# sebastianffx/stainlib

Hardware: AMD Instinct MI355X
Metric: 1024x1024 H&E tiles/sec normalized (Macenko) (higher is better)
Workload: dtype f32; 1 GPU; configs[1]: batch of 512 tiles 1024x1024x3 uint8 per GPU, Macenko transform (fit once outside the timed region), tiles resident in HBM; tiles_per_gpu=512, failed_tiles=0

## Files before the change

stainlib_amd/csrc/stats_finish.hpp:

```cpp
#pragma once
#include "stats_selection.hpp"
#include "stats_sweeps.hpp"

namespace sl {

struct SampleAngleKey {
    const uint32_t* sample; TabView tab; float V[6]; int cps_log2; int P; float ylimf;
    __device__ __forceinline__ float operator()(int b) const {
        if (sample_absent(b, cps_log2, P)) return nan_f();
        return of_word(sample[b]);
    }
    __device__ __forceinline__ float of_word(uint32_t s) const {
        const uint32_t r = s & 255u, g = (s >> 8) & 255u, bl = (s >> 16) & 255u;
        const bool tissue = is_tissue_f(tab.gam(r), tab.gam(g), tab.gam(bl), ylimf);
        const float k = angle_key(V, tab.odf(r), tab.odf(g), tab.odf(bl));
        return tissue ? k : nan_f();
    }
    __device__ __forceinline__ bool present(int b, int n_sample) const { return b < n_sample && !sample_absent(b, cps_log2, P); }
};
struct SampleConcKey {
    const uint32_t* sample; TabView tab; LassoK L; int cps_log2; int P; int col;
    __device__ __forceinline__ void both(int b, float& c1, float& c2) const {
        if (sample_absent(b, cps_log2, P)) { c1 = c2 = nan_f(); return; }
        of_word(sample[b], c1, c2);
// ... 173 lines not shown
        uint32_t best = 0xffffffffu;
        float kn[U];
#pragma unroll
        for (int u = 0; u < U; ++u) { const int i = tid + u * bd; kn[u] = as_global(cand)[i < n ? i : 0]; }
        for (int i0 = tid; i0 < n; i0 += U * bd) {
            float k[U];
#pragma unroll
            for (int u = 0; u < U; ++u) {
                k[u] = kn[u];
                const int i = i0 + (U + u) * bd;
                kn[u] = as_global(cand)[i < n ? i : 0];
            }
#pragma unroll
            for (int u = 0; u < U; ++u) {
                if (i0 + u * bd >= n) continue;
                const int kb = pick_bin(k[u], ps.lo[b], ps.sc[b]);
                if (kb == (int)bin[b]) { const uint32_t pos = atomicAdd(&S.misc[24 + b], 1u); if (pos < 512u) list[512 * b + pos] = k[u]; }
                else if (kb > (int)bin[b]) best = min(best, f2ord(k[u]));
            }
        }
        for (int o = 32; o > 0; o >>= 1) best = min(best, (uint32_t)__shfl_xor((int)best, o, 64));
        if (lane == 0 && best != 0xffffffffu) atomicMin(&S.misc[26 + b], best);
    }
    __syncthreads();
    if (tid < 4) S.misc[28 + tid] = 0;
    __syncthreads();
#pragma unroll
    for (int b = 0; b < 2; ++b) {
        if (!done[b]) continue;
        const uint32_t m = cnt[b], ra = krel[b] - below[b];
        if ((uint32_t)tid < m) {
            const float me = list[512 * b + tid];
            uint32_t r = 0;
            for (uint32_t j = 0; j < m; ++j) {
                const float o = list[512 * b + j];
                r += (o < me || (o == me && j < (uint32_t)tid)) ? 1u : 0u;
            }
            if (r == ra) S.misc[28 + 2 * b] = __float_as_uint(me);
            if (r == ra + 1) S.misc[29 + 2 * b] = __float_as_uint(me);
        }
    }
    __syncthreads();
#pragma unroll
    for (int b = 0; b < 2; ++b) {
        if (!done[b]) continue;
        xa[b] = __uint_as_float(S.misc[28 + 2 * b]);
        const bool same_bin = krel[b] - below[b] + 1 < cnt[b];
        const uint32_t nx = S.misc[26 + b];
        xb[b] = same_bin ? __uint_as_float(S.misc[29 + 2 * b]) : (nx != 0xffffffffu ? ord2f(nx) : xa[b]);
    }
    __syncthreads();
}

template <bool TWO_COLS, class TileKeyAt>
__device__ __forceinline__ void stage_pick2(const float* cand0, const float* cand1, const uint32_t* n_in, uint32_t cap_list, bool complete,
                                            const float* lo, const float* hi, const long long* lt, int P, TileKeyAt tile_key_at, uint32_t n,
                                            const long long* k, const PickScale& ps, float* res , int& fallbacks, SelScratch& S) {
    bool fast[2], has2[2];
    uint32_t krel[2];
#pragma unroll
    for (int b = 0; b < 2; ++b) {
        const long long k2 = (k[b] + 1 < (long long)n) ? k[b] + 1 : k[b];
        has2[b] = k2 != k[b];
        const bool covered = complete && k[b] >= lt[b] && k2 < lt[b] + (long long)n_in[b];
        fast[b] = covered && lo[b] < hi[b] && n_in[b] <= cap_list;
        krel[b] = fast[b] ? (uint32_t)(k[b] - lt[b]) : 0u;
    }
    float xa[2] = {0, 0}, xb[2] = {0, 0};
    bool done[2] = {false, false};
    if (fast[0] | fast[1]) wg_pick2(cand0, cand1, n_in, fast, krel, ps, xa, xb, done, S);
#pragma unroll
    for (int b = 0; b < 2; ++b) {
        if (done[b]) {
            if (!has2[b]) xb[b] = xa[b];
        } else {
            if constexpr (TWO_COLS) tile_key_at.col = b;
            stage_order_stats(b ? cand1 : cand0, n_in[b], cap_list, complete, lo[b], hi[b], lt[b], P, tile_key_at, n, k[b], xa[b], xb[b], fallbacks, S);
        }
        res[2 * b] = xa[b]; res[2 * b + 1] = xb[b];
    }
}

__device__ __noinline__ void raw_flush(uint32_t buf_lds, uint32_t n, uint32_t* dst, unsigned int* head, uint32_t cap) {
#if defined(__HIP_DEVICE_COMPILE__)
    SL_LDS const uint32_t* buf = (SL_LDS const uint32_t*)buf_lds;
#else
    const uint32_t* buf = nullptr;
#endif
    const int lane = threadIdx.x & 63;
    uint32_t base = 0;
    if (lane == 0) base = atomicAdd(head, n);
    base = __builtin_amdgcn_readfirstlane(base);
    for (uint32_t i = lane; i < n; i += 64)
        if (base + i < cap) as_global(dst)[base + i] = buf[i];
}

struct RawSink {
    uint32_t buf;
    uint32_t n;
    uint32_t* dst;
    unsigned int* head;
    unsigned int* overflow;
    uint32_t cap;
    uint32_t stage_cap;
    __device__ __forceinline__ void flush(int) {
        if (n != 0) raw_flush(buf, n, dst, head, cap);
        n = 0;
    }
    __device__ __forceinline__ void put(unsigned long long m, const Chunk& ch, int px, int lane) {
        put_value(m, chunk_pixel(ch, px) & 0xffffffu, lane);
    }
    __device__ __forceinline__ void put_value(unsigned long long m, uint32_t value, int lane) {
        const uint32_t cnt = (uint32_t)__popcll(m);
        if (__builtin_expect(n + cnt > stage_cap, 0)) flush(lane);
        const uint32_t rank = __builtin_amdgcn_mbcnt_hi((uint32_t)(m >> 32), __builtin_amdgcn_mbcnt_lo((uint32_t)m, 0u));
#if defined(__HIP_DEVICE_COMPILE__)
        uint32_t sbase;
        asm("s_lshl2_add_u32 %0, %1, %2" : "=s"(sbase) : "s"(n), "s"(buf) : "scc");
        const uint32_t addr = sbase + 4u * rank;
        unsigned long long saved;
        asm volatile("s_mov_b64 %0, exec\n\ts_mov_b64 exec, %1\n\tds_write_b32 %2, %3\n\ts_mov_b64 exec, %0"
                     : "=&s"(saved) : "s"(m), "v"(addr), "v"(value) : "memory");
#else
        (void)rank; (void)value;
#endif
        n += cnt;
    }
};


// ... 211 lines not shown
```

stainlib_amd/csrc/stats_fused.hpp:

```cpp
#pragma once
#include "stats_phase_kernels.hpp"
#include "stats_cube.hpp"
#include "stats_twosweep.hpp"

namespace sl {

struct FusedArgs {
    const uint8_t* rgb;
    uint8_t* out;
    int n_tiles;
    int P;
    int stride_log2;
    int n_sample;
    float ylimf;
    double lam;
    double pct;
    const double* M_tgt;
    const double* maxC_tgt;
    int cap_raw, cap_list;
    uint32_t* raw;
    int cap_ang;
    uint32_t* raw_ang;
    float* cand;
    uint32_t* sample;
// ... 12 lines not shown
    int32_t* sweeps_out;
    int use_cube;
    int32_t* cube_out;
    int two_sweep;
    int sample_cap;
    int cl_lines;
    int cl_scale_log2;
    int32_t* ts_out;
    unsigned long long* next_tile;
};

template <int NT>
struct FusedShared {
    RowTab tab;
    uint32_t stage[NT / 64][kStageWave];
    SelScratch S;
    alignas(8) unsigned int n_raw;
    unsigned int n_ang;
    unsigned int overflow;
    double red[NT / 64][32];
    double sum[32];
    DictIter it;
    double Vd[6];
    double M[6];
    double maxC[2];
    float Vf[6];
    float lo[2], hi[2];
    float box[4];
    float res[4];
    LassoK L;
    int status;
    int conc_done;
    float xmin;
    int why;
    int use_cube;
    MergedConc mk;
    TwoSweep ts;
    int next_tile;
};

template <int NT>
struct FusedLds {
    static constexpr uint32_t tab = 0u;
    static constexpr uint32_t stage = (uint32_t)sizeof(RowTab);
    static constexpr uint32_t stage_wave = 4u * (uint32_t)kStageWave;
    static constexpr uint32_t hist = (uint32_t)(sizeof(RowTab) + sizeof(uint32_t) * (NT / 64) * kStageWave);
};
template <int NT>
__device__ __forceinline__ void fused_lds_origin(const FusedShared<NT>& sh) {
    static_assert(offsetof(FusedShared<NT>, tab) == FusedLds<NT>::tab && offsetof(FusedShared<NT>, stage) == FusedLds<NT>::stage &&
                  offsetof(FusedShared<NT>, S) == FusedLds<NT>::hist && offsetof(SelScratch, hist) == 0, "");
    if (lds_address(&sh) != 0u) __builtin_trap();
}

#define SL_FINISH_ATTR __noinline__
#ifdef SL_DEBUG_SUBCLK
#define SL_SUB_AT(clk, j) { __syncthreads(); if ((clk) && tid == 0) (clk)[(j)] = wall_clock64(); }
#else
#define SL_SUB_AT(clk, j)
#endif
#define SL_SUB(j) SL_SUB_AT(subclk, j)
template <class T>
__device__ __forceinline__ T* uni_ptr(T* p) {
    const unsigned long long v = (unsigned long long)(uintptr_t)p;
    const uint32_t lo = (uint32_t)__builtin_amdgcn_readfirstlane((int)(uint32_t)v), hi = (uint32_t)__builtin_amdgcn_readfirstlane((int)(uint32_t)(v >> 32));
    return (T*)(uintptr_t)(((unsigned long long)hi << 32) | lo);
}
__device__ __forceinline__ double uni_d(double x) {
    const unsigned long long v = (unsigned long long)__double_as_longlong(x);
    const uint32_t lo = (uint32_t)__builtin_amdgcn_readfirstlane((int)(uint32_t)v), hi = (uint32_t)__builtin_amdgcn_readfirstlane((int)(uint32_t)(v >> 32));
    return __longlong_as_double((long long)(((unsigned long long)hi << 32) | lo));
}

template <int NT>
__device__ SL_FINISH_ATTR void fused_cube_build(FusedShared<NT>* shp, uint32_t* samp_, int n_sample_, int cps_log2_, int P_, float ylimf_, int want_cube_) {
    FusedShared<NT>& sh = *shp;
    uint32_t* samp = uni_ptr(samp_);
    const int n_sample = __builtin_amdgcn_readfirstlane(n_sample_), cps_log2 = __builtin_amdgcn_readfirstlane(cps_log2_), P = __builtin_amdgcn_readfirstlane(P_);
    const int want_cube = __builtin_amdgcn_readfirstlane(want_cube_);
    const float ylimf = uni(ylimf_);
    const int tid = threadIdx.x;
    float* ctab = reinterpret_cast<float*>(&sh.stage[0][0]);
    static_assert(sizeof(sh.stage) >= sizeof(float) * kCubeTabFloats && sizeof(sh.S.hist) >= 4 * kCubeWords, "");
    const CubeConsts cc = cube_tables(view_of_b(sh.tab), sh.Vf, sh.hi[0], sh.lo[1], sh.mk, ctab, tid);
    __syncthreads();
    int share_pct;
    const bool pays = cube_worthwhile<NT>(samp, n_sample, cps_log2, P, ctab, cc, ylimf, &sh.S.misc[33], tid, share_pct);
    const bool go = pays || want_cube == 2;
    if (tid == 0) sh.use_cube = (go ? 1 : 0) | (share_pct << 8);
    if (go) cube_mask<NT>(ctab, cc, ylimf, sh.S.hist, tid);
    __syncthreads();
}

template <int NT>
__device__ SL_FINISH_ATTR void fused_finish1(FusedShared<NT>* shp, uint32_t* samp_, int n_sample_, int stride_log2_, int P_, float ylimf_, double pct_, double lam_,
                                           long long* subclk_, int want_cube_) {
    FusedShared<NT>& sh = *shp;
    uint32_t* samp = uni_ptr(samp_);
    const int n_sample = __builtin_amdgcn_readfirstlane(n_sample_), P = __builtin_amdgcn_readfirstlane(P_);
    const int sl2 = __builtin_amdgcn_readfirstlane(stride_log2_);
    const bool dense = sl2 < 0;
    const int stride_log2 = dense ? -sl2 : sl2;
    const int cps_log2 = dense ? kDenseCps : stride_log2 - 2;
    const float zs = dense ? (float)sqrt(kClusterDeff) : 1.0f;
    const int want_cube = __builtin_amdgcn_readfirstlane(want_cube_);
    const float ylimf = uni(ylimf_);
// ... 175 lines not shown
                                               float ylimf_, int stream_) {
    FusedShared<NT>& sh = *shp;
    const uint8_t* src = uni_ptr(src_);
    uint32_t* rawl = uni_ptr(rawl_);
    uint32_t* rawa = uni_ptr(rawa_);
    const int P = __builtin_amdgcn_readfirstlane(P_), cap_raw = __builtin_amdgcn_readfirstlane(cap_raw_), stream = __builtin_amdgcn_readfirstlane(stream_);
    const int cap_ang = __builtin_amdgcn_readfirstlane(cap_ang_);
    const float ylimf = uni(ylimf_);
    const int tid = threadIdx.x, wave = tid >> 6;
    const TabReaderB TB = TabReaderB::make_at(FusedLds<NT>::tab);
    const int nch = (P + 3) >> 2;
    SelConsts K;
    for (int i = 0; i < 6; ++i) K.V[i] = in_vgpr(sh.Vf[i]);
    K.L.g12 = 0.0f;
    K.xmin = -INFINITY;
#pragma unroll
    for (int i = 0; i < 2; ++i) {
        K.u[i][0] = in_vgpr(sh.mk.u[i][0]); K.u[i][1] = in_vgpr(sh.mk.u[i][1]); K.kt[i] = in_vgpr(sh.mk.kt[i]);
        K.eps[i] = in_vgpr(sh.mk.eps[i]); K.thr[i] = in_vgpr(sh.mk.thr[i]);
    }
    K.lo0 = uni(sh.lo[0]); K.hi0 = uni(sh.hi[0]); K.lo1 = uni(sh.lo[1]); K.hi1 = uni(sh.hi[1]);
    static_assert(offsetof(FusedShared<NT>, n_ang) == offsetof(FusedShared<NT>, n_raw) + 4 && offsetof(FusedShared<NT>, n_raw) % 8 == 0, "");
    const RawDirect direct{rawl, rawa, reinterpret_cast<unsigned long long*>(&sh.n_raw), (uint32_t)cap_raw, (uint32_t)cap_ang};
    static_assert(offsetof(FusedShared<NT>, S) % 4096 == 0 && offsetof(SelScratch, hist) == 0, "the cube mask must be 4 KB aligned");
    const uint32_t bits_lds = FusedLds<NT>::hist;
    const uint32_t ring_lds = (uint32_t)__builtin_amdgcn_readfirstlane((int)(FusedLds<NT>::stage + (uint32_t)wave * FusedLds<NT>::stage_wave));
    int t, c0, c1;
    fused_geometry<NT>(nch, tid, t, c0, c1);
    if (c0 >= c1) return;
    if (stream) select_sweep_cube<ALIGNED, kFusedTrip, true>(src, P, c0, c1, t, kFusedThreads, TB, ylimf, K, bits_lds, ring_lds, direct);
    else select_sweep_cube<ALIGNED, kFusedTrip, false>(src, P, c0, c1, t, kFusedThreads, TB, ylimf, K, bits_lds, ring_lds, direct);
}

template <int NT>
__device__ SL_FINISH_ATTR int fused_finish2(FusedShared<NT>* shp, const uint8_t* src_, uint32_t* rawl_, uint32_t* rawa_, float* cand0_, float* cand1_, int P_,
                                          int cap_raw_, int cap_ang_, int cap_list_, float ylimf_, double pct_, double lam_, long long* subclk_, int ts_ = 0) {
    FusedShared<NT>& sh = *shp;
    const uint8_t* src = uni_ptr(src_);
    uint32_t* rawl = uni_ptr(rawl_);
    uint32_t* rawa = uni_ptr(rawa_);
    const int cap_ang = __builtin_amdgcn_readfirstlane(cap_ang_);
    float* cand0 = uni_ptr(cand0_);
    float* cand1 = uni_ptr(cand1_);
    const int P = __builtin_amdgcn_readfirstlane(P_), cap_raw = __builtin_amdgcn_readfirstlane(cap_raw_), cap_list = __builtin_amdgcn_readfirstlane(cap_list_);
    const float ylimf = uni(ylimf_);
    const double pct = uni_d(pct_), lam = uni_d(lam_);
    long long* subclk = uni_ptr(subclk_);
    const int ts = __builtin_amdgcn_readfirstlane(ts_);
    const int tid = threadIdx.x, wave = tid >> 6;
    int fallbacks = 0;
    (void)subclk;
    const uint32_t T = (uint32_t)sh.sum[0];
    long long k[2];
    double gfrac[2];
    percentile_pos((double)T, 100.0 - pct, k[0], gfrac[0]);
    percentile_pos((double)T, pct, k[1], gfrac[1]);
    fin_tab_build(sh.tab);
    const FinTab FT{FusedLds<NT>::tab};
    const uint32_t stage_lds = FusedLds<NT>::tab + kFinTabBytes + (uint32_t)wave * fin_stage_bytes(NT);
    const uint32_t stage_entries = fin_stage_bytes(NT) / 8u;
    AngleTileKey tkey;
    tkey.src = src; tkey.tab = FT.view(); tkey.ylimf = ylimf;
    WordAngleKey rkey;
    rkey.T = FT; rkey.ylimf = ylimf;
    for (int i = 0; i < 6; ++i) { tkey.V[i] = sh.Vf[i]; rkey.V[i] = sh.Vf[i]; }
    const bool complete = sh.n_raw <= (uint32_t)cap_raw && sh.overflow == 0;
    const uint32_t n_raw = sh.n_raw < (uint32_t)cap_raw ? sh.n_raw : (uint32_t)cap_raw;
    const bool split = rawa != nullptr;
    const bool complete_a = split ? sh.n_ang <= (uint32_t)cap_ang : complete;
    const uint32_t n_a = split ? (sh.n_ang < (uint32_t)cap_ang ? sh.n_ang : (uint32_t)cap_ang) : n_raw;
    const uint32_t* lista = split ? rawa : rawl;
    const float los[2] = {sh.lo[0], sh.lo[1]}, his[2] = {sh.hi[0], sh.hi[1]};
    SL_SUB(2);
    const RefineOut ra = wg_refine_s(lista, (int)n_a, rkey, los[0], his[0], los[1], his[1], cand0, cand1, (uint32_t)cap_list, stage_lds,
                                     stage_entries, sh.S);
    SL_SUB(3);
    {
        const long long lt[2] = {(long long)ra.n_lt[0], (long long)T - (long long)ra.n_valid + (long long)ra.n_lt[1]};
        if (ts) {
            bool covered = complete_a;
#pragma unroll
            for (int b = 0; b < 2; ++b) {
                const long long k2 = (k[b] + 1 < (long long)T) ? k[b] + 1 : k[b];
                covered = covered & (k[b] >= lt[b]) & (k2 < lt[b] + (long long)ra.n_in[b]) & (ra.n_in[b] <= (uint32_t)cap_list);
            }
            if (!covered) {
                fin_tab_expand<NT>(sh.tab);
                return -1;
            }
        }
        float res[4];
        stage_pick2<false>(cand0, cand1, ra.n_in, (uint32_t)cap_list, complete_a, los, his, lt, P, tkey, T, k, ra.ps, res, fallbacks, sh.S);
        if (tid == 0) { sh.res[0] = res[0]; sh.res[1] = res[1]; sh.res[2] = res[2]; sh.res[3] = res[3]; }
        __syncthreads();
    }
    SL_SUB(5);
    if (tid < 64) {
        double M[6];
        stain_matrix_from_angles(sh.Vd, sh.res, gfrac, M, tid);
        if (tid == 0) {
            for (int i = 0; i < 6; ++i) sh.M[i] = M[i];
            if (stain_matrix_singular(M)) sh.status = SL_TILE_DEGENERATE_COV;
            const bool use = sh.status == SL_TILE_OK && complete && merged_verify(sh.mk, M, lam);
            sh.conc_done = use ? 1 : 0;
            sh.why = use ? 0 : (!sh.mk.ok ? SL_RESWEEP_NO_BOX : (!complete ? SL_RESWEEP_LIST_FULL : SL_RESWEEP_OUTSIDE_BOX));
            if (use) { LassoK L; lasso_consts(M, lam, L); sh.L = L; }
        }
    }
    __syncthreads();
    SL_SUB(6);
    if (sh.conc_done) {
        long long kc;
        double gc;
        percentile_pos((double)P, 99.0, kc, gc);
        const long long kc2 = kc + 1 < (long long)P ? kc + 1 : kc;
        WordConcKey ckey2;
        ckey2.T = FT; ckey2.L = sh.L;
        const float cl[2] = {sh.mk.L[0], sh.mk.L[1]}, chh[2] = {sh.mk.H[0], sh.mk.H[1]};
        const RefineOut rc = wg_refine_s(rawl, (int)n_raw, ckey2, cl[0], chh[0], cl[1], chh[1], cand0, cand1, (uint32_t)cap_list,
                                         stage_lds, stage_entries, sh.S);
        SL_SUB(14);
#ifdef SL_DEBUG_SUBCLK
        if (subclk && tid == 0) {
            long long* q = subclk;
            q[8] = 100ll * n_a; q[9] = 100ll * n_raw; q[10] = 100ll * (ra.n_in[0] + ra.n_in[1]); q[11] = 100ll * (rc.n_in[0] + rc.n_in[1]);
        }
#endif
        const long long n_plain = (long long)P - (long long)sh.n_raw;
        const long long clt[2] = {n_plain + rc.n_lt[0], n_plain + rc.n_lt[1]};
        bool covered = true;
#pragma unroll
        for (int col = 0; col < 2; ++col)
            covered = covered & (kc >= clt[col]) & (kc2 < clt[col] + (long long)rc.n_in[col]) & (rc.n_in[col] <= (uint32_t)cap_list);
        if (covered) {
            ConcTileKey ctk;
            ctk.src = src; ctk.tab = FT.view(); ctk.L = sh.L; ctk.col = 0;
            const long long kk[2] = {kc, kc};
            float res[4];
            stage_pick2<true>(cand0, cand1, rc.n_in, (uint32_t)cap_list, true, cl, chh, clt, P, ctk, (uint32_t)P, kk, rc.ps, res, fallbacks, sh.S);
            if (tid == 0) {
                sh.maxC[0] = np_lerp((double)res[0], (double)res[1], gc);
                sh.maxC[1] = np_lerp((double)res[2], (double)res[3], gc);
                if (!(sh.maxC[0] > 0.0) || !(sh.maxC[1] > 0.0)) sh.status = SL_TILE_ZERO_MAXC;
            }
        } else if (tid == 0) {
            sh.conc_done = 0;
            sh.why = (rc.n_in[0] > (uint32_t)cap_list || rc.n_in[1] > (uint32_t)cap_list) ? SL_RESWEEP_LIST_FULL : SL_RESWEEP_BRACKET_MISSED;
        }
        __syncthreads();
        SL_SUB(15);
    }
    fin_tab_expand<NT>(sh.tab);
    return fallbacks;
}

template <int NT>
__device__ __noinline__ void phase0_estimate(FusedShared<NT>* shp, int mode_) {
    FusedShared<NT>& sh = *shp;
    const int mode = __builtin_amdgcn_readfirstlane(mode_);
    double Vd[6], wv[3];
    float Vf[6];
    const int st = eigvecs_from_moments(sh.sum, Vd, Vf, wv);
    const double ns = sh.sum[0];
    const double l1 = wv[0], l2 = wv[1], l3 = wv[2] > 0.0 ? wv[2] : 0.0;
    bool ok = st == SL_TILE_OK && ns >= (double)kTsMinTissue && l2 > 1e-9 * l1 && l2 - l3 > 0.05 * l2;
    double tau = 0.0;
    if (ok) {
        tau = kTiltZ * sqrt(kClusterDeff / ns) * fmax(sqrt(l3 * l2) / (l2 - l3), sqrt(l3 * l1) / (l1 - l3));
        tau = fmax(tau, kTsMinTau);
        ok = tau <= (mode >= 2 ? kTsMaxTau : kTsAutoMaxTau);
    }
    double nd[3] = {Vd[2] * Vd[5] - Vd[4] * Vd[3], Vd[4] * Vd[1] - Vd[0] * Vd[5], Vd[0] * Vd[3] - Vd[2] * Vd[1]};
    const double nn = 1.0 / sqrt(nd[0] * nd[0] + nd[1] * nd[1] + nd[2] * nd[2]);
    if (mode == 4 && ok) {
        double b[3];
        for (int c = 0; c < 3; ++c) b[c] = Vd[2 * c + 1] + 0.05 * nd[c] * nn;
        const double nb = 1.0 / sqrt(b[0] * b[0] + b[1] * b[1] + b[2] * b[2]);
        for (int c = 0; c < 3; ++c) { Vd[2 * c + 1] = b[c] * nb; Vf[2 * c + 1] = (float)Vd[2 * c + 1]; }
        nd[0] = Vd[2] * Vd[5] - Vd[4] * Vd[3]; nd[1] = Vd[4] * Vd[1] - Vd[0] * Vd[5]; nd[2] = Vd[0] * Vd[3] - Vd[2] * Vd[1];
    }
    const double nn2 = 1.0 / sqrt(nd[0] * nd[0] + nd[1] * nd[1] + nd[2] * nd[2]);
    for (int i = 0; i < 6; ++i) { sh.ts.Vd[i] = Vd[i]; sh.Vd[i] = Vd[i]; sh.Vf[i] = Vf[i]; }
    for (int c = 0; c < 3; ++c) { sh.ts.nd[c] = nd[c] * nn2; sh.ts.fn[c] = (float)(nd[c] * nn2); }
    sh.ts.tau = tau;
    sh.ts.gH[0] = l1 - l3; sh.ts.gH[1] = l2 - l3;
    sh.res[0] = (float)(4.0 * sqrt(l3));
    sh.res[1] = (float)(sh.sum[1] / ns); sh.res[2] = (float)(sh.sum[2] / ns); sh.res[3] = (float)(sh.sum[3] / ns);
    sh.status = ok ? SL_TILE_OK : SL_TILE_DEGENERATE_COV;
}

template <int NT>
__device__ __noinline__ void phase0_cone_and_box(FusedShared<NT>* shp, float hi0_, float lo1_, double lam_) {
    FusedShared<NT>& sh = *shp;
    const float hi0 = uni(hi0_), lo1 = uni(lo1_);
    const double lam = uni_d(lam_);
    const int tid = threadIdx.x;
    const double aH = angle_of_pseudo((double)hi0), aL = angle_of_pseudo((double)lo1);
    double sH, cH, sL, cL;
    sincos(aH, &sH, &cH);
    sincos(aL, &sL, &cL);
    if (tid == 0) {
        const double k2 = sh.ts.kappa2 + 6e-6;
        for (int c = 0; c < 3; ++c) {
            const double gH = sh.ts.Vd[2 * c] * -sH + sh.ts.Vd[2 * c + 1] * cH, gL = sh.ts.Vd[2 * c] * sL + sh.ts.Vd[2 * c + 1] * -cL;
            sh.ts.gH[c] = gH; sh.ts.gL[c] = gL;
            sh.ts.fgH[c] = (float)(gH - k2); sh.ts.fgL[c] = (float)(gL - k2);
        }
        sh.ts.fk1 = (float)(sh.ts.kappa1 * (1.0 + 1e-6));
        sh.ts.lo0 = sh.lo[0]; sh.ts.hi1 = sh.hi[1];
    }
    ts_box(sh.ts.Vd, sh.ts.nd, sh.ts.tau, sh.box, lam, tid, sh.mk);
}

constexpr int kP0Bins = 1024;
template <int NT>
__device__ SL_FINISH_ATTR void fused_phase0(FusedShared<NT>* shp, const uint8_t* src_, uint32_t* samp_, int P_, int n_lines_, float ylimf_, double pct_, double lam_,
                                          int mode_, int cap_raw_, int cap_ang_, int cap_list_, long long* subclk_) {
    FusedShared<NT>& sh = *shp;
    const uint8_t* src = uni_ptr(src_);
    uint32_t* samp = uni_ptr(samp_);
    const int P = __builtin_amdgcn_readfirstlane(P_), n_lines = __builtin_amdgcn_readfirstlane(n_lines_), mode = __builtin_amdgcn_readfirstlane(mode_);
    const int cap_raw = __builtin_amdgcn_readfirstlane(cap_raw_), cap_ang = __builtin_amdgcn_readfirstlane(cap_ang_), cap_list = __builtin_amdgcn_readfirstlane(cap_list_);
    const float ylimf = uni(ylimf_);
    const double pct = uni_d(pct_), lam = uni_d(lam_);
    long long* subclk = uni_ptr(subclk_);
    const int tid = threadIdx.x, lane = tid & 63, wave = tid >> 6;
    const int n_sample = n_lines * kClusterPx;
    constexpr int KPT = kMaxSample / NT;
    static_assert(KPT % 8 == 0, "");
    (void)subclk;
    SL_SUB(0);
    if (tid == 0) { sh.ts.ok = 0; sh.ts.why = kTsNoEstimate; sh.mk.ok = 0; sh.use_cube = 0; }
    const TabView tab = view_of_b(sh.tab);
    uint32_t w[KPT];
    Moments mo;
    BurstMoments bm;
    double cnt = 0.0;
    {
        const uint32_t nl = (uint32_t)(((3ll * P) >> 7) < 1 ? 1 : ((3ll * P) >> 7));
        const uint32_t wl = nl / (uint32_t)n_lines;
#pragma unroll
        for (int j0 = 0; j0 < KPT; j0 += 8) {
#pragma unroll
            for (int u = 0; u < 8; ++u) {
                const int b = min((j0 + u) * NT + tid, n_sample - 1);
                w[j0 + u] = cluster_word(src, P, wl, (uint32_t)b);
            }
#pragma unroll
            for (int u = 0; u < 8; ++u) {
                const int b = (j0 + u) * NT + tid;
                if (b < n_sample) {
                    as_global(samp)[b] = w[j0 + u];
                    const uint32_t r = w[j0 + u] & 255u, g = (w[j0 + u] >> 8) & 255u, bl = (w[j0 + u] >> 16) & 255u;
                    if (is_tissue_f(tab.gam(r), tab.gam(g), tab.gam(bl), ylimf)) {
                        bm.add(tab.odf(r), tab.odf(g), tab.odf(bl));
                        cnt += 1.0;
                    }
                }
            }
        }
        bm.flush(mo);
    }
    {
        double v[10];
        mo.to_array(v, 0u, lane);
        v[0] = cnt;
#pragma unroll
        for (int i = 0; i < 10; ++i) v[i] = wave_sum(v[i]);
        if (lane == 0)
            for (int i = 0; i < 10; ++i) sh.red[wave][i] = v[i];
    }
    for (int i = tid; i < kP0Bins; i += NT) sh.S.hist[i] = 0;
    __syncthreads();
    SL_SUB(1);
    if (tid < 10) {
        double t = 0;
        for (int wv = 0; wv < NT / 64; ++wv) t += sh.red[wv][tid];
        sh.sum[tid] = t;
    }
    __syncthreads();
    if (tid == 0) phase0_estimate<NT>(shp, mode);
    __syncthreads();
    SL_SUB(2);
    if (sh.status != SL_TILE_OK) return;
    {
        float V[6], nf[3];
        for (int i = 0; i < 6; ++i) V[i] = sh.Vf[i];
        for (int c = 0; c < 3; ++c) nf[c] = sh.ts.fn[c];
        const float mx = sh.res[1], my = sh.res[2], mz = sh.res[3];
        float q1 = 0.0f, q2 = 0.0f;
#pragma unroll
        for (int j = 0; j < KPT; ++j) {
            const int b = j * NT + tid;
            const uint32_t r = w[j] & 255u, g = (w[j] >> 8) & 255u, bl = (w[j] >> 16) & 255u;
            const float ox = tab.odf(r), oy = tab.odf(g), oz = tab.odf(bl);
            const bool tissue = (b < n_sample) & is_tissue_f(tab.gam(r), tab.gam(g), tab.gam(bl), ylimf);
            if (tissue) {
                const float key = angle_key(V, ox, oy, oz);
                const int bin = min(kP0Bins - 1, max(0, (int)((key + 1.0f) * (0.5f * kP0Bins))));
                atomicAdd(&sh.S.hist[bin], 1u);
                const float dx = ox - mx, dy = oy - my, dz = oz - mz;
                const float a1 = fmaf(V[4], dz, fmaf(V[2], dy, V[0] * dx)), a2 = fmaf(V[5], dz, fmaf(V[3], dy, V[1] * dx));
                const float a3 = fmaf(nf[2], dz, fmaf(nf[1], dy, nf[0] * dx));
                q1 = fmaf(a1 * a3, a1 * a3, q1);
                q2 = fmaf(a2 * a3, a2 * a3, q2);
            }
        }
        double d1 = wave_sum((double)q1), d2 = wave_sum((double)q2);
        if (lane == 0) { sh.red[wave][0] = d1; sh.red[wave][1] = d2; }
    }
    __syncthreads();
    {
        const double n = sh.sum[0];
        const double zsd = sqrt(kClusterDeff);
        if (wave < 8) {
            const int which = wave & 3, b = which >> 1, upper = which & 1;
            const double q = (b == 0 ? 100.0 - pct : pct) / 100.0;
            const double z = (wave < 4 ? (double)kBracketZ : (double)kBoxZ) * zsd;
            const double r = q * (n - 1.0), sd = sqrt(fmax(q * (1.0 - q) * n, 0.0));
            const long long rk = upper ? (long long)ceil(r + z * sd) + 1 : (long long)floor(r - z * sd) - 1;
            const bool open = upper ? rk > (long long)n - 1 : rk < 0;
            uint32_t* o = &sh.S.misc[kLocateOut - 24 + 3 * wave];
            if (!open) wave_locate(sh.S.hist, kP0Bins, (uint32_t)rk, o, lane);
            else if (lane == 0) o[0] = 0xffffffffu;
        }
        if (tid == 0) {
            double t1 = 0.0, t2 = 0.0;
            for (int wv = 0; wv < NT / 64; ++wv) { t1 += sh.red[wv][0]; t2 += sh.red[wv][1]; }
            const double se = fmax(sqrt(t1) / (n * sh.ts.gH[0]), sqrt(t2) / (n * sh.ts.gH[1]));
            const double tau = fmax(sh.ts.tau, kTiltZ4 * sqrt(kClusterDeff) * se);
            sh.ts.tau = tau;
            sh.ts.kappa1 = tau;
            sh.ts.kappa2 = tau * tau + 1e-7;
            if (!(tau <= kTsMaxTau)) sh.status = SL_TILE_DEGENERATE_COV;
        }
    }
    __syncthreads();
    if (tid == 0) {
        float e[8];
        for (int i = 0; i < 8; ++i) {
            const uint32_t bin = sh.S.misc[kLocateOut - 24 + 3 * i];
            const bool upper = i & 1;
            const bool open = bin == 0xffffffffu || bin == 0u || bin >= (uint32_t)(kP0Bins - 1);
            e[i] = open ? (upper ? INFINITY : -INFINITY) : -1.0f + (float)(bin + (upper ? 1u : 0u)) * (2.0f / kP0Bins);
        }
        sh.lo[0] = e[0]; sh.hi[0] = e[1]; sh.lo[1] = e[2]; sh.hi[1] = e[3];
        const bool closed = (e[0] > -INFINITY) & (e[1] < INFINITY) & (e[2] > -INFINITY) & (e[3] < INFINITY);
        if (closed) {
            for (int b = 0; b < 2; ++b) {
                const float m = 0.5f * (e[2 * b] + e[2 * b + 1]), r = (float)kBoxFrac * 0.5f * (e[2 * b + 1] - e[2 * b]);
                sh.box[2 * b] = m - r; sh.box[2 * b + 1] = m + r;
            }
        } else {
            for (int i = 0; i < 4; ++i) sh.box[i] = e[4 + i];
        }
    }
    for (int i = tid; i < kP0Bins; i += NT) sh.S.hist[i] = 0;
    __syncthreads();
    SL_SUB(3);
    if (sh.status != SL_TILE_OK) return;
    const float hi0 = sh.hi[0], lo1 = sh.lo[1];
    if (!(hi0 > -0.95f && hi0 < lo1 && lo1 < 0.95f)) return;
    if (tid < 64) phase0_cone_and_box<NT>(shp, hi0, lo1, lam);
    __syncthreads();
    SL_SUB(4);
    if (sh.mk.ok) {
        LassoK L = sh.mk.Lc;
        uint32_t nz1 = 0, nz2 = 0;
#pragma unroll
        for (int j = 0; j < KPT; ++j) {
            const int b = j * NT + tid;
            float c1, c2;
            lasso2(L, tab.odf(w[j] & 255u), tab.odf((w[j] >> 8) & 255u), tab.odf((w[j] >> 16) & 255u), c1, c2);
            const int b1 = min(511, max(0, (int)(512.0f * c1 * __builtin_amdgcn_rcpf(c1 + 1.0f))));
            const int b2 = min(511, max(0, (int)(512.0f * c2 * __builtin_amdgcn_rcpf(c2 + 1.0f))));
            const bool in = b < n_sample;
            const unsigned long long z1 = __builtin_amdgcn_ballot_w64(in & (b1 == 0)), z2 = __builtin_amdgcn_ballot_w64(in & (b2 == 0));
            if (in & (b1 != 0)) atomicAdd(&sh.S.hist[b1], 1u);
            if (in & (b2 != 0)) atomicAdd(&sh.S.hist[512 + b2], 1u);
            nz1 += (uint32_t)__popcll(z1); nz2 += (uint32_t)__popcll(z2);
        }
        if (lane == 0) { if (nz1) atomicAdd(&sh.S.hist[0], nz1); if (nz2) atomicAdd(&sh.S.hist[512], nz2); }
        __syncthreads();
        if (wave < 4) {
            const int col = wave >> 1, upper = wave & 1;
            const double n = (double)n_sample, q = 0.99;
            const double z = (double)kBracketZ * sqrt(kClusterDeff);
            const double r = q * (n - 1.0), sd = sqrt(q * (1.0 - q) * n);
            const long long rk = upper ? (long long)ceil(r + z * sd) + 1 : (long long)floor(r - z * sd) - 1;
            const bool open = upper ? rk > (long long)n - 1 : rk < 0;
            uint32_t* o = &sh.S.misc[kLocateOut - 24 + 3 * wave];
            if (!open) wave_locate(sh.S.hist + 512 * col, 512, (uint32_t)rk, o, lane);
            else if (lane == 0) o[0] = 0xffffffffu;
        }
        __syncthreads();
        if (tid == 0) {
            float e[4];
            for (int i = 0; i < 4; ++i) {
                const uint32_t bin = sh.S.misc[kLocateOut - 24 + 3 * i];
                const bool upper = i & 1;
                const bool open = bin == 0xffffffffu || (upper && bin >= 511u);
                const float edge = (float)(bin + (upper ? 1u : 0u));
                e[i] = open ? (upper ? INFINITY : -INFINITY) : (upper ? edge / (512.0f - edge) * (1.0f + 1e-5f) : edge / (512.0f - edge) * (1.0f - 1e-5f));
            }
            ts_thresholds(sh.mk, e[0], e[2], e[1], e[3], sh.res[0]);
        }
    }
    __syncthreads();
    SL_SUB(7);
    if (!sh.mk.ok && mode < 2) return;
    if (!sh.mk.ok && tid == 0) ts_thresholds(sh.mk, -INFINITY, -INFINITY, -INFINITY, -INFINITY, 0.0f);
    if (tid == 0) {
        for (int i = 0; i < 2; ++i) {
            for (int c = 0; c < 3; ++c) sh.ts.W[i][c] = sh.mk.ok ? (float)sh.mk.C.W[i][c] : 0.0f;
            sh.ts.kt[i] = sh.mk.kt[i]; sh.ts.eps[i] = sh.mk.eps[i]; sh.ts.zeta[i] = (float)(sh.mk.zeta[i] * (1.0 + 1e-6)); sh.ts.thr[i] = sh.mk.thr[i];
        }
        sh.S.misc[34] = 0; sh.S.misc[35] = 0;
    }
    __syncthreads();
    if (sh.mk.ok) {
        if (wave < 2) {
            const float ref = (sh.mk.H[0] < INFINITY ? sh.mk.H[0] : 2.0f * sh.mk.L[0] + 1.0f) + (sh.mk.H[1] < INFINITY ? sh.mk.H[1] : 2.0f * sh.mk.L[1] + 1.0f);
            const float cut = fmaxf(sh.mk.thr[wave] - sh.mk.eps[wave] * ref - (float)sh.mk.zeta[wave] * sh.res[0], 0.0f);
            const int bl = min(511, max(0, (int)(512.0f * cut / (cut + 1.0f))));
            uint32_t cntm = 0;
            for (int b = lane; b < 512; b += 64) cntm += b >= bl ? sh.S.hist[512 * wave + b] : 0u;
            for (int o = 32; o > 0; o >>= 1) cntm += (uint32_t)__shfl_xor((int)cntm, o, 64);
            if (lane == 0) atomicAdd(&sh.S.misc[35], cntm);
        }
        __syncthreads();
        const double scale = (double)P / (double)n_sample;
        const bool full = (double)sh.S.misc[35] * scale > 0.75 * (double)cap_raw || (double)sh.S.misc[35] * scale > 1.5 * (double)cap_list;
        if (full && mode < 2) {
            if (tid == 0) sh.ts.why = kTsLists;
            return;
        }
    }
    (void)cap_ang;
    SL_SUB(5);
    {
        float* ctab = reinterpret_cast<float*>(&sh.stage[0][0]);
        static_assert(sizeof(sh.stage) >= sizeof(float) * kTsTabFloats, "");
        const TsCubeConsts cc = ts_cube_tables(view_of_b(sh.tab), sh.ts, ctab, tid);
        if (tid == 0) sh.S.misc[33] = 0;
        __syncthreads();
        uint32_t amb = 0, seen = 0;
#pragma unroll
        for (int j = 0; j < KPT; j += KPT / 2) {
            if (j * NT + tid < n_sample) {
                amb += ts_cell_plain(ctab, cc, ylimf, w[j]) ? 0u : 1u;
                ++seen;
            }
        }
        uint32_t both = amb | (seen << 16);
        for (int o = 32; o > 0; o >>= 1) both += (uint32_t)__shfl_xor((int)both, o, 64);
        if (lane == 0 && both) atomicAdd(&sh.S.misc[33], both);
        __syncthreads();
        const uint32_t tot = sh.S.misc[33];
        const int share = (tot >> 16) ? (int)(100u * (tot & 0xffffu) / (tot >> 16)) : 100;
        const bool go = share <= kTsMaxSharePct || mode >= 2;
        if (tid == 0) {
            sh.use_cube = (go ? 1 : 0) | (share << 8);
            sh.ts.ok = go ? 1 : 0;
            sh.ts.why = go ? kTsDirect : kTsShare;
        }
        if (go) ts_cube_mask<NT>(ctab, cc, ylimf, sh.S.hist, tid);
        __syncthreads();
    }
    SL_SUB(6);
}

template <int NT, bool ALIGNED>
__device__ __noinline__ void fused_sweep1c(FusedShared<NT>* shp, const uint8_t* src_, uint32_t* rawl_, uint32_t* rawa_, int P_, int cap_raw_, int cap_ang_,
                                           float ylimf_, int stream_) {
    FusedShared<NT>& sh = *shp;
    const uint8_t* src = uni_ptr(src_);
    uint32_t* rawl = uni_ptr(rawl_);
    uint32_t* rawa = uni_ptr(rawa_);
    const int P = __builtin_amdgcn_readfirstlane(P_), cap_raw = __builtin_amdgcn_readfirstlane(cap_raw_), stream = __builtin_amdgcn_readfirstlane(stream_);
    const int cap_ang = __builtin_amdgcn_readfirstlane(cap_ang_);
    const float ylimf = uni(ylimf_);
    const int tid = threadIdx.x, lane = tid & 63, wave = tid >> 6;
    const TabReaderB TB = TabReaderB::make_at(FusedLds<NT>::tab);
    const int nch = (P + 3) >> 2;
    TsSweepConsts K;
#define SL_TSK(x) uni(x)
#pragma unroll
    for (int c = 0; c < 3; ++c) { K.gH[c] = SL_TSK(sh.ts.fgH[c]); K.gL[c] = SL_TSK(sh.ts.fgL[c]); K.n[c] = SL_TSK(sh.ts.fn[c]); }
    K.k1 = SL_TSK(sh.ts.fk1);
#pragma unroll
    for (int i = 0; i < 2; ++i) {
#pragma unroll
        for (int c = 0; c < 3; ++c) K.W[i][c] = SL_TSK(sh.ts.W[i][c]);
        K.kt[i] = SL_TSK(sh.ts.kt[i]); K.eps[i] = SL_TSK(sh.ts.eps[i]); K.zeta[i] = SL_TSK(sh.ts.zeta[i]); K.thr[i] = uni(sh.ts.thr[i]);
    }
#undef SL_TSK
    const RawDirect direct{rawl, rawa, reinterpret_cast<unsigned long long*>(&sh.n_raw), (uint32_t)cap_raw, (uint32_t)cap_ang};
    const uint32_t bits_lds = FusedLds<NT>::hist;
    const uint32_t ring_lds = (uint32_t)__builtin_amdgcn_readfirstlane((int)(FusedLds<NT>::stage + (uint32_t)wave * FusedLds<NT>::stage_wave));
    Moments mo;
    uint32_t n_tissue = 0;
    int t, c0, c1;
    fused_geometry<NT>(nch, tid, t, c0, c1);
// ... 393 lines not shown
```

stainlib_amd/csrc/stats_linalg.hpp:

```cpp
#pragma once
#include "stats_common.hpp"

namespace sl {

__device__ __forceinline__ void jacobi_rot(double& app, double& aqq, double& apq, double& apr, double& aqr,
                                           double (&vp)[3], double (&vq)[3]) {
    if (apq == 0.0) return;
    const double theta = (aqq - app) / (2.0 * apq);
    const double t = (theta >= 0 ? 1.0 : -1.0) / (fabs(theta) + sqrt(theta * theta + 1.0));
    const double c = 1.0 / sqrt(t * t + 1.0), sn = t * c;
    app -= t * apq;
    aqq += t * apq;
    apq = 0.0;
    const double npr = c * apr - sn * aqr, nqr = sn * apr + c * aqr;
    apr = npr;
    aqr = nqr;
#pragma unroll
    for (int i = 0; i < 3; ++i) {
        const double a = vp[i], b = vq[i];
        vp[i] = c * a - sn * b;
        vq[i] = sn * a + c * b;
    }
}

// ... 4 lines not shown
    double a00 = 0, a01 = 0, a02 = 0, a11 = 0, a12 = 0, a22 = 0;
    if (n < 1) status = SL_TILE_EMPTY_MASK;
    else if (n < 2) status = SL_TILE_DEGENERATE_COV;
    else {
        const double mx = sum[1] / n, my = sum[2] / n, mz = sum[3] / n, inv = 1.0 / (n - 1.0);
        a00 = (sum[4] - n * mx * mx) * inv; a01 = (sum[5] - n * mx * my) * inv; a02 = (sum[6] - n * mx * mz) * inv;
        a11 = (sum[7] - n * my * my) * inv; a12 = (sum[8] - n * my * mz) * inv; a22 = (sum[9] - n * mz * mz) * inv;
        for (int sweep = 0; sweep < 30; ++sweep) {
            const double off = fabs(a01) + fabs(a02) + fabs(a12);
            const double dia = fabs(a00) + fabs(a11) + fabs(a22);
            if (off <= 1e-300 || off <= 1e-22 * dia) break;
            jacobi_rot(a00, a11, a01, a02, a12, v0, v1);
            jacobi_rot(a00, a22, a02, a01, a12, v0, v2);
            jacobi_rot(a11, a22, a12, a01, a02, v1, v2);
        }
    }
    double w0 = a00, w1 = a11, w2 = a22;
#define SL_SWAP_COL(wa, wb, va, vb) do { const double tw = wa; wa = wb; wb = tw; \
        for (int i_ = 0; i_ < 3; ++i_) { const double tv = va[i_]; va[i_] = vb[i_]; vb[i_] = tv; } } while (0)
    if (w0 > w1) SL_SWAP_COL(w0, w1, v0, v1);
    if (w1 > w2) SL_SWAP_COL(w1, w2, v1, v2);
    if (w0 > w1) SL_SWAP_COL(w0, w1, v0, v1);
#undef SL_SWAP_COL
    if (status == SL_TILE_OK) {
        const double scale = (sum[4] + sum[7] + sum[9]) / n;
        if (!(w2 > 1e-12 * scale)) {
            v2[0] = 1; v2[1] = 0; v2[2] = 0; v1[0] = 0; v1[1] = 1; v1[2] = 0;
        } else if (!(w1 > 1e-12 * scale)) {
            int ax = 0;
            if (fabs(v2[1]) < fabs(v2[ax])) ax = 1;
            if (fabs(v2[2]) < fabs(v2[ax])) ax = 2;
            double u[3] = {-v2[ax] * v2[0], -v2[ax] * v2[1], -v2[ax] * v2[2]};
            u[ax] += 1.0;
            const double nu = sqrt(u[0] * u[0] + u[1] * u[1] + u[2] * u[2]);
            for (int i = 0; i < 3; ++i) v1[i] = u[i] / nu;
        }
    }
    if (w_out) { w_out[0] = w2; w_out[1] = w1; w_out[2] = w0; }
    const double s2 = v2[0] < 0 ? -1.0 : 1.0, s1 = v1[0] < 0 ? -1.0 : 1.0;
#pragma unroll
    for (int c = 0; c < 3; ++c) {
        Vd[c * 2 + 0] = s2 * v2[c]; Vf[c * 2 + 0] = (float)(s2 * v2[c]);
        Vd[c * 2 + 1] = s1 * v1[c]; Vf[c * 2 + 1] = (float)(s1 * v1[c]);
    }
    return status;
}

__device__ __forceinline__ bool stain_matrix_singular(const double* M) {
    const double g11 = M[0] * M[0] + M[1] * M[1] + M[2] * M[2], g22 = M[3] * M[3] + M[4] * M[4] + M[5] * M[5];
    const double g12 = M[0] * M[3] + M[1] * M[4] + M[2] * M[5];
    return !(g11 * g22 - g12 * g12 > 1e-8 * g11 * g22);
}

__device__ __forceinline__ void stain_matrix_from_angles(const double* Vd, const float* xs , const double* gfrac, double* M, int lane) {
    const double ang = angle_of_pseudo((double)xs[lane & 3]);
    const int pair = (lane & 1) * 2;
    const double phi = np_lerp(__shfl(ang, pair, 64), __shfl(ang, pair + 1, 64), (lane & 1) ? gfrac[1] : gfrac[0]);
    double s, c;
    sincos(phi, &s, &c);
    const double s1 = __shfl(s, 0, 64), c1 = __shfl(c, 0, 64), s2 = __shfl(s, 1, 64), c2 = __shfl(c, 1, 64);
    double v1[3], v2[3];
#pragma unroll
    for (int c = 0; c < 3; ++c) {
        v1[c] = Vd[c * 2] * c1 + Vd[c * 2 + 1] * s1;
        v2[c] = Vd[c * 2] * c2 + Vd[c * 2 + 1] * s2;
    }
    const bool first = v1[0] > v2[0];
    double h[3], e[3];
#pragma unroll
    for (int c = 0; c < 3; ++c) { h[c] = first ? v1[c] : v2[c]; e[c] = first ? v2[c] : v1[c]; }
    const double nh = sqrt(h[0] * h[0] + h[1] * h[1] + h[2] * h[2]);
    const double ne = sqrt(e[0] * e[0] + e[1] * e[1] + e[2] * e[2]);
#pragma unroll
    for (int c = 0; c < 3; ++c) { M[c] = h[c] / nh; M[3 + c] = e[c] / ne; }
}

constexpr double kBoxFrac = 0.6;
constexpr double kBoxInflate = 1.25;
constexpr double kBoxMaxEps = 0.25;

struct LassoD { double W[2][3], k[2], g12; };
__device__ __forceinline__ void lasso_affine_d(const double* M, double lam, LassoD& o) {
    const double g11 = M[0] * M[0] + M[1] * M[1] + M[2] * M[2];
    const double g22 = M[3] * M[3] + M[4] * M[4] + M[5] * M[5];
    const double g12 = M[0] * M[3] + M[1] * M[4] + M[2] * M[5];
    const double det = g11 * g22 - g12 * g12;
    const double i11 = g22 / det, i12 = -g12 / det, i22 = g11 / det;
#pragma unroll
    for (int c = 0; c < 3; ++c) {
        o.W[0][c] = i11 * M[c] + i12 * M[3 + c];
        o.W[1][c] = i12 * M[c] + i22 * M[3 + c];
    }
    o.k[0] = -lam * (i11 + i12);
    o.k[1] = -lam * (i12 + i22);
    o.g12 = g12;
}
__device__ __forceinline__ void relate_affine(const LassoD& A, const LassoD& C, double (&T)[2][2], double (&r)[2]) {
    double g[2][2], b[2][2];
#pragma unroll
    for (int i = 0; i < 2; ++i)
#pragma unroll
        for (int j = 0; j < 2; ++j) {
            g[i][j] = C.W[i][0] * C.W[j][0] + C.W[i][1] * C.W[j][1] + C.W[i][2] * C.W[j][2];
            b[i][j] = A.W[i][0] * C.W[j][0] + A.W[i][1] * C.W[j][1] + A.W[i][2] * C.W[j][2];
        }
    const double rd = 1.0 / (g[0][0] * g[1][1] - g[0][1] * g[1][0]);
#pragma unroll
    for (int i = 0; i < 2; ++i) {
        T[i][0] = (b[i][0] * g[1][1] - b[i][1] * g[1][0]) * rd;
        T[i][1] = (b[i][1] * g[0][0] - b[i][0] * g[0][1]) * rd;
        r[i] = A.k[i] - T[i][0] * C.k[0] - T[i][1] * C.k[1];
    }
}
__device__ __forceinline__ void stain_matrix_from_phi(const double* Vd, double phi_min, double phi_max, double* M) {
    double s1, c1, s2, c2;
    sincos(phi_min, &s1, &c1);
    sincos(phi_max, &s2, &c2);
    double v1[3], v2[3];
#pragma unroll
    for (int c = 0; c < 3; ++c) {
        v1[c] = Vd[c * 2] * c1 + Vd[c * 2 + 1] * s1;
        v2[c] = Vd[c * 2] * c2 + Vd[c * 2 + 1] * s2;
    }
    const bool first = v1[0] > v2[0];
    double h[3], e[3];
#pragma unroll
    for (int c = 0; c < 3; ++c) { h[c] = first ? v1[c] : v2[c]; e[c] = first ? v2[c] : v1[c]; }
// ... 118 lines not shown
```

Baseline: 371,600 tiles/s.

## Cut register pressure in fused stats kernel via cold calls and streamed sample rows

```diff
diff --git a/stainlib_amd/csrc/stats_finish.hpp b/stainlib_amd/csrc/stats_finish.hpp
--- a/stainlib_amd/csrc/stats_finish.hpp
+++ b/stainlib_amd/csrc/stats_finish.hpp
@@ -249,9 +249,17 @@
     __syncthreads();
 }
 
-template <bool TWO_COLS, class TileKeyAt>
+struct ColdStats { float xa, xb; int fallbacks; };
+template <class MakeTileKey>
+__device__ __noinline__ ColdStats stage_order_stats_cold(const float* cand, uint32_t n_in, uint32_t cap_list, int complete, float lo, float hi, long long lt, int P,
+                                                         MakeTileKey make_tile_key, int b, uint32_t n, long long k, SelScratch* S) {
+    ColdStats r{0.0f, 0.0f, 0};
+    stage_order_stats(cand, n_in, cap_list, complete != 0, lo, hi, lt, P, make_tile_key(b), n, k, r.xa, r.xb, r.fallbacks, *S);
+    return r;
+}
+template <class MakeTileKey>
 __device__ __forceinline__ void stage_pick2(const float* cand0, const float* cand1, const uint32_t* n_in, uint32_t cap_list, bool complete,
-                                            const float* lo, const float* hi, const long long* lt, int P, TileKeyAt tile_key_at, uint32_t n,
+                                            const float* lo, const float* hi, const long long* lt, int P, MakeTileKey make_tile_key, uint32_t n,
                                             const long long* k, const PickScale& ps, float* res , int& fallbacks, SelScratch& S) {
     bool fast[2], has2[2];
     uint32_t krel[2];
@@ -271,8 +279,8 @@
         if (done[b]) {
             if (!has2[b]) xb[b] = xa[b];
         } else {
-            if constexpr (TWO_COLS) tile_key_at.col = b;
-            stage_order_stats(b ? cand1 : cand0, n_in[b], cap_list, complete, lo[b], hi[b], lt[b], P, tile_key_at, n, k[b], xa[b], xb[b], fallbacks, S);
+            const ColdStats c = stage_order_stats_cold(b ? cand1 : cand0, n_in[b], cap_list, complete ? 1 : 0, lo[b], hi[b], lt[b], P, make_tile_key, b, n, k[b], &S);
+            xa[b] = c.xa; xb[b] = c.xb; fallbacks += c.fallbacks;
         }
         res[2 * b] = xa[b]; res[2 * b + 1] = xb[b];
     }
diff --git a/stainlib_amd/csrc/stats_fused.hpp b/stainlib_amd/csrc/stats_fused.hpp
--- a/stainlib_amd/csrc/stats_fused.hpp
+++ b/stainlib_amd/csrc/stats_fused.hpp
@@ -88,6 +88,7 @@
                   offsetof(FusedShared<NT>, S) == FusedLds<NT>::hist && offsetof(SelScratch, hist) == 0, "");
     if (lds_address(&sh) != 0u) __builtin_trap();
 }
+static_assert(sizeof(FusedShared<kFusedThreads>) <= 81920, "two 512-thread workgroups share a CU's 160 KB of LDS");
 
 #define SL_FINISH_ATTR __noinline__
 #ifdef SL_DEBUG_SUBCLK
@@ -369,18 +370,24 @@
     (void)subclk;
     const uint32_t T = (uint32_t)sh.sum[0];
     long long k[2];
-    double gfrac[2];
-    percentile_pos((double)T, 100.0 - pct, k[0], gfrac[0]);
-    percentile_pos((double)T, pct, k[1], gfrac[1]);
+    {
+        double g;
+        percentile_pos((double)T, 100.0 - pct, k[0], g);
+        percentile_pos((double)T, pct, k[1], g);
+    }
     fin_tab_build(sh.tab);
     const FinTab FT{FusedLds<NT>::tab};
     const uint32_t stage_lds = FusedLds<NT>::tab + kFinTabBytes + (uint32_t)wave * fin_stage_bytes(NT);
     const uint32_t stage_entries = fin_stage_bytes(NT) / 8u;
-    AngleTileKey tkey;
-    tkey.src = src; tkey.tab = FT.view(); tkey.ylimf = ylimf;
+    const auto tile_angle_key = [shp, src, ylimf](int) {
+        AngleTileKey tkey;
+        tkey.src = src; tkey.tab = FinTab{FusedLds<NT>::tab}.view(); tkey.ylimf = ylimf;
+        for (int i = 0; i < 6; ++i) tkey.V[i] = shp->Vf[i];
+        return tkey;
+    };
     WordAngleKey rkey;
     rkey.T = FT; rkey.ylimf = ylimf;
-    for (int i = 0; i < 6; ++i) { tkey.V[i] = sh.Vf[i]; rkey.V[i] = sh.Vf[i]; }
+    for (int i = 0; i < 6; ++i) rkey.V[i] = sh.Vf[i];
     const bool complete = sh.n_raw <= (uint32_t)cap_raw && sh.overflow == 0;
     const uint32_t n_raw = sh.n_raw < (uint32_t)cap_raw ? sh.n_raw : (uint32_t)cap_raw;
     const bool split = rawa != nullptr;
@@ -407,14 +414,18 @@
             }
         }
         float res[4];
-        stage_pick2<false>(cand0, cand1, ra.n_in, (uint32_t)cap_list, complete_a, los, his, lt, P, tkey, T, k, ra.ps, res, fallbacks, sh.S);
+        stage_pick2(cand0, cand1, ra.n_in, (uint32_t)cap_list, complete_a, los, his, lt, P, tile_angle_key, T, k, ra.ps, res, fallbacks, sh.S);
         if (tid == 0) { sh.res[0] = res[0]; sh.res[1] = res[1]; sh.res[2] = res[2]; sh.res[3] = res[3]; }
         __syncthreads();
     }
     SL_SUB(5);
     if (tid < 64) {
         double M[6];
-        stain_matrix_from_angles(sh.Vd, sh.res, gfrac, M, tid);
+        long long kd;
+        double g0, g1;
+        percentile_pos((double)T, 100.0 - pct, kd, g0);
+        percentile_pos((double)T, pct, kd, g1);
+        stain_matrix_from_angles(sh.Vd, sh.res, g0, g1, M, tid);
         if (tid == 0) {
             for (int i = 0; i < 6; ++i) sh.M[i] = M[i];
             if (stain_matrix_singular(M)) sh.status = SL_TILE_DEGENERATE_COV;
@@ -450,11 +461,14 @@
         for (int col = 0; col < 2; ++col)
             covered = covered & (kc >= clt[col]) & (kc2 < clt[col] + (long long)rc.n_in[col]) & (rc.n_in[col] <= (uint32_t)cap_list);
         if (covered) {
-            ConcTileKey ctk;
-            ctk.src = src; ctk.tab = FT.view(); ctk.L = sh.L; ctk.col = 0;
+            const auto tile_conc_key = [shp, src](int col) {
+                ConcTileKey ctk;
+                ctk.src = src; ctk.tab = FinTab{FusedLds<NT>::tab}.view(); ctk.L = shp->L; ctk.col = col;
+                return ctk;
+            };
             const long long kk[2] = {kc, kc};
             float res[4];
-            stage_pick2<true>(cand0, cand1, rc.n_in, (uint32_t)cap_list, true, cl, chh, clt, P, ctk, (uint32_t)P, kk, rc.ps, res, fallbacks, sh.S);
+            stage_pick2(cand0, cand1, rc.n_in, (uint32_t)cap_list, true, cl, chh, clt, P, tile_conc_key, (uint32_t)P, kk, rc.ps, res, fallbacks, sh.S);
             if (tid == 0) {
                 sh.maxC[0] = np_lerp((double)res[0], (double)res[1], gc);
                 sh.maxC[1] = np_lerp((double)res[2], (double)res[3], gc);
@@ -528,6 +542,26 @@
     }
     ts_box(sh.ts.Vd, sh.ts.nd, sh.ts.tau, sh.box, lam, tid, sh.mk);
 }
+
+template <int NT>
+struct SampleRows {
+    const uint32_t* samp;
+    int n_sample, tid;
+    uint32_t nx[kBrkBatch];
+    __device__ __forceinline__ SampleRows(const uint32_t* s, int n, int t) : samp(s), n_sample(n), tid(t) {
+        asm volatile("" : "+v"(tid));
+        load(0);
+    }
+    __device__ __forceinline__ void load(int j0) {
+#pragma unroll
+        for (int u = 0; u < kBrkBatch; ++u) nx[u] = as_global(samp)[min((j0 + u) * NT + tid, n_sample - 1)];
+    }
+    __device__ __forceinline__ void next(uint32_t* w, int j0) {
+#pragma unroll
+        for (int u = 0; u < kBrkBatch; ++u) w[u] = nx[u];
+        if (j0 + kBrkBatch < kMaxSample / NT) load(j0 + kBrkBatch);
+    }
+};
 
 constexpr int kP0Bins = 1024;
 template <int NT>
@@ -549,7 +583,6 @@
     SL_SUB(0);
     if (tid == 0) { sh.ts.ok = 0; sh.ts.why = kTsNoEstimate; sh.mk.ok = 0; sh.use_cube = 0; }
     const TabView tab = view_of_b(sh.tab);
-    uint32_t w[KPT];
     Moments mo;
     BurstMoments bm;
     double cnt = 0.0;
@@ -557,18 +590,19 @@
         const uint32_t nl = (uint32_t)(((3ll * P) >> 7) < 1 ? 1 : ((3ll * P) >> 7));
         const uint32_t wl = nl / (uint32_t)n_lines;
 #pragma unroll
-        for (int j0 = 0; j0 < KPT; j0 += 8) {
-#pragma unroll
-            for (int u = 0; u < 8; ++u) {
+        for (int j0 = 0; j0 < KPT; j0 += kBrkBatch) {
+            uint32_t w[kBrkBatch];
+#pragma unroll
+            for (int u = 0; u < kBrkBatch; ++u) {
                 const int b = min((j0 + u) * NT + tid, n_sample - 1);
-                w[j0 + u] = cluster_word(src, P, wl, (uint32_t)b);
-            }
-#pragma unroll
-            for (int u = 0; u < 8; ++u) {
+                w[u] = cluster_word(src, P, wl, (uint32_t)b);
+            }
+#pragma unroll
+            for (int u = 0; u < kBrkBatch; ++u) {
                 const int b = (j0 + u) * NT + tid;
                 if (b < n_sample) {
-                    as_global(samp)[b] = w[j0 + u];
-                    const uint32_t r = w[j0 + u] & 255u, g = (w[j0 + u] >> 8) & 255u, bl = (w[j0 + u] >> 16) & 255u;
+                    as_global(samp)[b] = w[u];
+                    const uint32_t r = w[u] & 255u, g = (w[u] >> 8) & 255u, bl = (w[u] >> 16) & 255u;
                     if (is_tissue_f(tab.gam(r), tab.gam(g), tab.gam(bl), ylimf)) {
                         bm.add(tab.odf(r), tab.odf(g), tab.odf(bl));
                         cnt += 1.0;
@@ -606,21 +640,27 @@
         for (int c = 0; c < 3; ++c) nf[c] = sh.ts.fn[c];
         const float mx = sh.res[1], my = sh.res[2], mz = sh.res[3];
         float q1 = 0.0f, q2 = 0.0f;
-#pragma unroll
-        for (int j = 0; j < KPT; ++j) {
-            const int b = j * NT + tid;
-            const uint32_t r = w[j] & 255u, g = (w[j] >> 8) & 255u, bl = (w[j] >> 16) & 255u;
-            const float ox = tab.odf(r), oy = tab.odf(g), oz = tab.odf(bl);
-            const bool tissue = (b < n_sample) & is_tissue_f(tab.gam(r), tab.gam(g), tab.gam(bl), ylimf);
-            if (tissue) {
-                const float key = angle_key(V, ox, oy, oz);
-                const int bin = min(kP0Bins - 1, max(0, (int)((key + 1.0f) * (0.5f * kP0Bins))));
-                atomicAdd(&sh.S.hist[bin], 1u);
-                const float dx = ox - mx, dy = oy - my, dz = oz - mz;
-                const float a1 = fmaf(V[4], dz, fmaf(V[2], dy, V[0] * dx)), a2 = fmaf(V[5], dz, fmaf(V[3], dy, V[1] * dx));
-                const float a3 = fmaf(nf[2], dz, fmaf(nf[1], dy, nf[0] * dx));
-                q1 = fmaf(a1 * a3, a1 * a3, q1);
-                q2 = fmaf(a2 * a3, a2 * a3, q2);
+        SampleRows<NT> rows(samp, n_sample, tid);
+#pragma unroll
+        for (int j0 = 0; j0 < KPT; j0 += kBrkBatch) {
+            uint32_t w[kBrkBatch];
+            rows.next(w, j0);
+#pragma unroll
+            for (int u = 0; u < kBrkBatch; ++u) {
+                const int b = (j0 + u) * NT + tid;
+                const uint32_t r = w[u] & 255u, g = (w[u] >> 8) & 255u, bl = (w[u] >> 16) & 255u;
+                const float ox = tab.odf(r), oy = tab.odf(g), oz = tab.odf(bl);
+                const bool tissue = (b < n_sample) & is_tissue_f(tab.gam(r), tab.gam(g), tab.gam(bl), ylimf);
+                if (tissue) {
+                    const float key = angle_key(V, ox, oy, oz);
+                    const int bin = min(kP0Bins - 1, max(0, (int)((key + 1.0f) * (0.5f * kP0Bins))));
+                    atomicAdd(&sh.S.hist[bin], 1u);
+                    const float dx = ox - mx, dy = oy - my, dz = oz - mz;
+                    const float a1 = fmaf(V[4], dz, fmaf(V[2], dy, V[0] * dx)), a2 = fmaf(V[5], dz, fmaf(V[3], dy, V[1] * dx));
+                    const float a3 = fmaf(nf[2], dz, fmaf(nf[1], dy, nf[0] * dx));
+                    q1 = fmaf(a1 * a3, a1 * a3, q1);
+                    q2 = fmaf(a2 * a3, a2 * a3, q2);
+                }
             }
         }
         double d1 = wave_sum((double)q1), d2 = wave_sum((double)q2);
@@ -684,18 +724,24 @@
     if (sh.mk.ok) {
         LassoK L = sh.mk.Lc;
         uint32_t nz1 = 0, nz2 = 0;
-#pragma unroll
-        for (int j = 0; j < KPT; ++j) {
-            const int b = j * NT + tid;
-            float c1, c2;
-            lasso2(L, tab.odf(w[j] & 255u), tab.odf((w[j] >> 8) & 255u), tab.odf((w[j] >> 16) & 255u), c1, c2);
-            const int b1 = min(511, max(0, (int)(512.0f * c1 * __builtin_amdgcn_rcpf(c1 + 1.0f))));
-            const int b2 = min(511, max(0, (int)(512.0f * c2 * __builtin_amdgcn_rcpf(c2 + 1.0f))));
-            const bool in = b < n_sample;
-            const unsigned long long z1 = __builtin_amdgcn_ballot_w64(in & (b1 == 0)), z2 = __builtin_amdgcn_ballot_w64(in & (b2 == 0));
-            if (in & (b1 != 0)) atomicAdd(&sh.S.hist[b1], 1u);
-            if (in & (b2 != 0)) atomicAdd(&sh.S.hist[512 + b2], 1u);
-            nz1 += (uint32_t)__popcll(z1); nz2 += (uint32_t)__popcll(z2);
+        SampleRows<NT> rows(samp, n_sample, tid);
+#pragma unroll
+        for (int j0 = 0; j0 < KPT; j0 += kBrkBatch) {
+            uint32_t w[kBrkBatch];
+            rows.next(w, j0);
+#pragma unroll
+            for (int u = 0; u < kBrkBatch; ++u) {
+                const int b = (j0 + u) * NT + tid;
+                float c1, c2;
+                lasso2(L, tab.odf(w[u] & 255u), tab.odf((w[u] >> 8) & 255u), tab.odf((w[u] >> 16) & 255u), c1, c2);
+                const int b1 = min(511, max(0, (int)(512.0f * c1 * __builtin_amdgcn_rcpf(c1 + 1.0f))));
+                const int b2 = min(511, max(0, (int)(512.0f * c2 * __builtin_amdgcn_rcpf(c2 + 1.0f))));
+                const bool in = b < n_sample;
+                const unsigned long long z1 = __builtin_amdgcn_ballot_w64(in & (b1 == 0)), z2 = __builtin_amdgcn_ballot_w64(in & (b2 == 0));
+                if (in & (b1 != 0)) atomicAdd(&sh.S.hist[b1], 1u);
+                if (in & (b2 != 0)) atomicAdd(&sh.S.hist[512 + b2], 1u);
+                nz1 += (uint32_t)__popcll(z1); nz2 += (uint32_t)__popcll(z2);
+            }
         }
         if (lane == 0) { if (nz1) atomicAdd(&sh.S.hist[0], nz1); if (nz2) atomicAdd(&sh.S.hist[512], nz2); }
         __syncthreads();
@@ -765,7 +811,7 @@
 #pragma unroll
         for (int j = 0; j < KPT; j += KPT / 2) {
             if (j * NT + tid < n_sample) {
-                amb += ts_cell_plain(ctab, cc, ylimf, w[j]) ? 0u : 1u;
+                amb += ts_cell_plain(ctab, cc, ylimf, as_global(samp)[j * NT + tid]) ? 0u : 1u;
                 ++seen;
             }
         }
diff --git a/stainlib_amd/csrc/stats_linalg.hpp b/stainlib_amd/csrc/stats_linalg.hpp
--- a/stainlib_amd/csrc/stats_linalg.hpp
+++ b/stainlib_amd/csrc/stats_linalg.hpp
@@ -80,10 +80,10 @@
     return !(g11 * g22 - g12 * g12 > 1e-8 * g11 * g22);
 }
 
-__device__ __forceinline__ void stain_matrix_from_angles(const double* Vd, const float* xs , const double* gfrac, double* M, int lane) {
+__device__ __forceinline__ void stain_matrix_from_angles(const double* Vd, const float* xs , double g0, double g1, double* M, int lane) {
     const double ang = angle_of_pseudo((double)xs[lane & 3]);
     const int pair = (lane & 1) * 2;
-    const double phi = np_lerp(__shfl(ang, pair, 64), __shfl(ang, pair + 1, 64), (lane & 1) ? gfrac[1] : gfrac[0]);
+    const double phi = np_lerp(__shfl(ang, pair, 64), __shfl(ang, pair + 1, 64), (lane & 1) ? g1 : g0);
     double s, c;
     sincos(phi, &s, &c);
     const double s1 = __shfl(s, 0, 64), c1 = __shfl(c, 0, 64), s2 = __shfl(s, 1, 64), c2 = __shfl(c, 1, 64);
@@ -101,6 +101,9 @@
     const double ne = sqrt(e[0] * e[0] + e[1] * e[1] + e[2] * e[2]);
 #pragma unroll
     for (int c = 0; c < 3; ++c) { M[c] = h[c] / nh; M[3 + c] = e[c] / ne; }
+}
+__device__ __forceinline__ void stain_matrix_from_angles(const double* Vd, const float* xs , const double* gfrac, double* M, int lane) {
+    stain_matrix_from_angles(Vd, xs, gfrac[0], gfrac[1], M, lane);
 }
 
 constexpr double kBoxFrac = 0.6;
```

After: 380,800 tiles/s (median of 6 runs). 2.5% higher.
